# david8862/tf-keras-speech-commands

Hardware: AMD Instinct MI355X
Metric: 1 s@16 kHz clips/sec train-step, simple_cnn bs4096, 1/2/4/8 MI355X; eval top-1 (higher is better)
Workload: dtype f32; 1 GPU; configs[1]: simple_cnn train step = featurize(f32 1 s @16 kHz) + fwd + bwd + Adam, 36 logits (background + 35 words), batch 4096 per GPU; global_batch=4096, parallelism=dp1, gradient_exchange=none (one rank), rccl_ranks=0, library_build=546ca62dfe01

## Files before the change

### tf-keras-speech-commands_amd/csrc/kws_cnn_plan.h

```cpp
#pragma once
#include "kws_model_types.h"
#include "kws_layers.h"
#include "kws_layer1.h"
#include "kws_infer_fused.h"
#include "kws_conv_group.h"
#include "kws_dense_head.h"
#include "kws_conv.h"
#include "kws_conv2_wgrad_fast.h"

namespace kws {

struct CnnPlan {
    bool training, bf16, det;
    bool prepared;
    bool fused_tail;
    bool group;
    bool dense_fused;
    bool l1m;
    bool l1_default_map;
    bool prep_in_stats;
    bool l1_conv2;
    bool compact_g2;
    bool routed_g2;
    bool fuse_pool2;
    bool acc_fwd;
    bool acc_bn2, acc_bn3, acc_bn4;
    bool a3_on_load;
    bool pool4_fused;
    bool wgrad2_bf16;
    bool wgrad2_early;
    bool wgrad2_fast;
    bool l1_fin_in_kernel;
    bool head_bwd_fuses;
    bool fuse_head_fwd;
};

inline CnnPlan plan_cnn(const kws_model *m, int B, int mprec, bool training, bool capturing, bool wants_head_outputs, bool prepared)
{
    const CnnDims &d = m->d;
    CnnPlan p{};
    p.training = training;
    p.bf16 = mprec == 1;
    p.det = m->deterministic != 0;
    p.prepared = !training && prepared;
    const bool split_train = p.bf16 && training;
    const bool default_tail = m->kind == KWS_SIMPLE_CNN && d.H2 == kFuH2 && d.W2 == kFuW2 && d.H3 == kFuH3 && d.W3 == kFuW3;
    p.fused_tail = !training && wants_head_outputs && p.bf16 && default_tail && d.H4 == kFuH4 && d.W4 == kFuW4 && m->C <= kFuHeadCols;
    p.group = split_train && default_tail && (long)blocks_for(B, kFuClips) <= kStatStride;
    p.head_bwd_fuses = head_bwd_fuses(m);
    p.fuse_head_fwd = p.head_bwd_fuses && !p.det;
    p.dense_fused = split_train && m->kind == KWS_SIMPLE_CNN && p.fuse_head_fwd && m->head_K == kDhK && d.flat % (16 * kDhWaves) == 0 && d.flat <= 1024;
    p.l1m = d.H0 % 2 == 0 && d.W0 % 2 == 0 && (d.H0 + 2) * (d.W0 + 2) <= 64 * kL1Stage && (d.H0 / 2) * (d.W0 / 2) <= 4 * kL1MaxTiles;
    p.l1_default_map = d.H0 == 30 && d.W0 == 20;
    p.prep_in_stats = split_train && p.l1m;
    const int P1 = d.H1 * d.W1;
    p.compact_g2 = p.bf16 && P1 * 8 <= 1280 && (size_t)(d.H1 / 2) * (d.W1 / 2) * 32 <= sizeof(float) * (size_t)d.H3 * d.W3 * 64;
    p.routed_g2 = p.compact_g2;
    p.fuse_pool2 = p.group && p.routed_g2 && d.H1 == kGrH1 && d.W1 == kGrW1;
    const bool acc_ok = !p.det && !capturing;
    p.acc_fwd = p.fuse_pool2 && acc_ok;
    p.l1_conv2 = p.prep_in_stats && p.acc_fwd && p.l1_default_map;
    p.a3_on_load = split_train;
    p.pool4_fused = p.acc_fwd && p.dense_fused;
    p.wgrad2_bf16 = p.bf16 && P1 <= 160;
    p.wgrad2_early = p.compact_g2 && p.wgrad2_bf16 && P1 * 8 <= 1280 && P1 * 4 <= 768;
    p.acc_bn2 = p.group && acc_ok && p.routed_g2 && p.wgrad2_early;
    p.acc_bn3 = p.group && acc_ok;
    p.acc_bn4 = p.dense_fused && acc_ok && d.flat == d.H4 * d.W4 * kDhK;
    p.l1_fin_in_kernel = acc_ok && p.l1_default_map;
    p.wgrad2_fast = p.wgrad2_early && p.acc_bn2 && d.H1 == kW2fH && d.W1 == kW2fW;
    return p;
}

}
```

### tf-keras-speech-commands_amd/csrc/kws_conv.h

```cpp
#pragma once
#include "kws_device.h"

namespace kws {

struct ConvGeom {
    int B, H, W, Ho, Wo;
    int stride, pt, pl;
    int KH, KW;
    int pmajor = 0;
};

enum { EPI_NONE = 0, EPI_RELU = 1, EPI_BIAS_RELU6 = 2, EPI_BIAS = 3, EPI_BIAS_RELU = 4,
       EPI_BN_RELU6 = 5,
       EPI_BNBWD_GATE6 = 6 };
enum { MODE_FWD = 0, MODE_DGRAD = 1 };

__host__ __device__ constexpr int stride16(int c) { return (c % 32 == 16) ? c : c + 16; }

template <int CR, int CO, int MODE, int EPI>
__global__ __launch_bounds__(256) void conv_gemm_kernel(const float *__restrict__ src, const float *__restrict__ wgt,
                                                         const float *__restrict__ bias, float *__restrict__ dst,
                                                         ConvGeom g)
{
    constexpr int KC = CR >= 32 ? 32 : CR;
// ... 332 lines not shown
            __syncthreads();
            store_chunk(s1, chunk + 1);
            __syncthreads();
            if (chunk + 3 < nchunks) load_chunk(chunk + 3, s1);
            mma_chunk();
        }
    }

    long mrow[RT][4];
#pragma unroll
    for (int rt = 0; rt < RT; ++rt)
#pragma unroll
        for (int r = 0; r < 4; ++r) {
            const long q = m0 + 16 * (wm * RT + rt) + 4 * lq + r;
            long m = q < M ? q : -1;
            if (pm && q < M) {
                int b, pix;
                row_of(q, b, pix);
                m = (long)b * P + pix;
            }
            mrow[rt][r] = m;
        }
    float ssum[CT], ssq[CT];
#pragma unroll
    for (int c = 0; c < CT; ++c) {
        const int n = 16 * (wn * CT + c) + li;
        float bv = 0.f, sv = 0.f;
        ssum[c] = 0.f; ssq[c] = 0.f;
        if (EPI == EPI_BIAS_RELU6 || EPI == EPI_BIAS || EPI == EPI_BIAS_RELU || EPI == EPI_BN_RELU6) bv = bias[n];
        if (EPI == EPI_BN_RELU6) sv = shift[n];
        float gsc = 0.f, gsh = 0.f, gmean = 0.f, ginv = 0.f;
        if (EPI == EPI_BNBWD_GATE6) { gsc = bias[n]; gsh = bias[CO + n]; gmean = bias[2 * CO + n]; ginv = bias[3 * CO + n]; }
#pragma unroll
        for (int rt = 0; rt < RT; ++rt)
#pragma unroll
            for (int r = 0; r < 4; ++r) {
                const long m = mrow[rt][r];
                if (m >= 0) {
                    float v = acc[rt][c][r];
                    if (EPI == EPI_RELU) v = fmaxf(v, 0.f);
                    if (EPI == EPI_BIAS_RELU6) v = relu6f(v + bv);
                    if (EPI == EPI_BIAS) v = v + bv;
                    if (EPI == EPI_BIAS_RELU) v = fmaxf(v + bv, 0.f);
                    if (EPI == EPI_BN_RELU6) v = relu6f(fmaf(v, bv, sv));
                    if (EPI == EPI_BNBWD_GATE6) {
                        const float zv = shift[m * CO + n], y = fmaf(zv, gsc, gsh);
                        v = (y > 0.f && y < 6.f) ? v : 0.f;
                        dst[m * CO + n] = v;
                        if (STATS) { ssum[c] += v; ssq[c] = fmaf(v, (zv - gmean) * ginv, ssq[c]); }
                        continue;
                    }
                    dst[m * CO + n] = v;
                    if (STATS) { ssum[c] += v; ssq[c] = fmaf(v, v, ssq[c]); }
                }
            }
    }
    if (STATS) {
        __syncthreads();
        double *red = reinterpret_cast<double *>(&As[0][0]);
#pragma unroll
        for (int c = 0; c < CT; ++c) {
            double a = (double)ssum[c], q = (double)ssq[c];
            a += __shfl_xor(a, 16, 64); a += __shfl_xor(a, 32, 64);
            q += __shfl_xor(q, 16, 64); q += __shfl_xor(q, 32, 64);
            const int n = 16 * (wn * CT + c) + li;
            if (lq == 0) { red[(wm * 2 + 0) * CO + n] = a; red[(wm * 2 + 1) * CO + n] = q; }
        }
        __syncthreads();
        for (int i = tid; i < 2 * CO; i += 256) {
            const int which = i / CO, n = i % CO;
            partial[((long)which * CO + n) * partial_stride + blockIdx.x] = red[(0 * 2 + which) * CO + n] + red[(1 * 2 + which) * CO + n];
        }
    }
}

__host__ __device__ constexpr int tr_row_words(int C) { return ((C / 2 / 8) & 1) ? C / 2 : C / 2 + 8; }

typedef short s16x4 __attribute__((ext_vector_type(4)));
__device__ __forceinline__ s16x4 lds_read_tr16(const unsigned char *p)
{
    return __builtin_amdgcn_ds_read_tr16_b64_v4i16((__attribute__((address_space(3))) s16x4 *)(p));
}

template <int CIN, int COUT, int TPB, bool DPRE = false, bool XBN = false>
__global__ __launch_bounds__(256, 2) void conv_wgrad_bf16_kernel(const float *__restrict__ x, const float *__restrict__ dzp,
                                                                  float *__restrict__ dw, const float *__restrict__ zero_page,
                                                                  ConvGeom g, int chunks_per_block, int nranges,
                                                                  Bf16Planes dpl = Bf16Planes{{nullptr, nullptr, nullptr}},
                                                                  const float *__restrict__ xbn = nullptr)
{
    constexpr int KC = 32;
    constexpr int XS = 4 * tr_row_words(CIN), DS = 4 * tr_row_words(COUT);
    constexpr int MT = CIN / 16, NT = COUT / 16, NW = NT / 4;
    constexpr int XU = KC * CIN / 4, DU = KC * COUT / 4;
    constexpr int NXU = XU / 256, NDU = DPRE ? DU / 2 / 256 : DU / 256;
    constexpr int XT = 3 * KC * XS;
    typedef unsigned u32x4 __attribute__((ext_vector_type(4)));
    static_assert(COUT % 64 == 0 && CIN % 32 == 0, "four waves split COUT in 16-column tiles; every thread stages whole units");
    extern __shared__ __attribute__((aligned(16))) unsigned char wsm[];
    unsigned char *Xs = wsm;
    unsigned char *Ds = wsm + TPB * XT;
    const int tid = threadIdx.x, lane = tid & 63, wave = tid >> 6, li = lane & 15, lq = lane >> 4;
    const int HW = g.Ho * g.Wo;
    const long M = (long)g.B * HW;
    const int ngroups = g.KH * g.KW / TPB;
    const int bid = blockIdx.x, tap0 = ((bid >> 3) % ngroups) * TPB, range = (bid / (8 * ngroups)) * 8 + (bid & 7);
    const long nchunk_all = (M + KC - 1) / KC, chunk0 = (long)range * chunks_per_block;
    const int nchunks = (range >= nranges || chunk0 >= nchunk_all) ? 0
                        : (int)(chunk0 + chunks_per_block <= nchunk_all ? chunks_per_block : nchunk_all - chunk0);

    f32x4 acc[TPB][MT][NW];
#pragma unroll
    for (int t = 0; t < TPB; ++t)
#pragma unroll
        for (int mt = 0; mt < MT; ++mt)
#pragma unroll
            for (int nw = 0; nw < NW; ++nw) acc[t][mt][nw] = (f32x4){0.f, 0.f, 0.f, 0.f};

    const float rWo = 1.0f / (float)g.Wo;
    int xb[NXU], xpix[NXU];
#pragma unroll
    for (int j = 0; j < NXU; ++j) {
        const long m = chunk0 * KC + (tid + 256 * j) / (CIN / 4);
        xb[j] = (int)(m / HW); xpix[j] = (int)(m - (long)xb[j] * HW);
    }
    f32x4 sx[TPB][NXU], sd[DPRE ? 1 : NDU];
    u32x4 sdp[DPRE ? 3 : 1][NDU];
    unsigned xok = 0u;
    f32x4 xsc = {0.f, 0.f, 0.f, 0.f}, xsh = {0.f, 0.f, 0.f, 0.f};
    if constexpr (XBN) {
        static_assert(256 % (CIN / 4) == 0 && NXU * TPB <= 32, "one channel group per thread");
        xsc = *reinterpret_cast<const f32x4 *>(xbn + 4 * (tid % (CIN / 4)));
        xsh = *reinterpret_cast<const f32x4 *>(xbn + CIN + 4 * (tid % (CIN / 4)));
    }
    auto load_chunk = [&](int ch) {
        const long m0 = (chunk0 + ch) * KC;
        xok = 0u;
#pragma unroll
        for (int j = 0; j < NXU; ++j) {
            const int e = (tid + 256 * j) % (CIN / 4);
            const int oy = (int)(((float)xpix[j] + 0.5f) * rWo), ox = xpix[j] - oy * g.Wo;
#pragma unroll
            for (int t = 0; t < TPB; ++t) {
                const int tap = tap0 + t, kh = tap / g.KW, kw = tap - kh * g.KW;
                const int sy = oy * g.stride + kh - g.pt, sxx = ox * g.stride + kw - g.pl;
                const bool ok = xb[j] < g.B && sy >= 0 && sy < g.H && sxx >= 0 && sxx < g.W;
                const float *p = ok ? x + (((long)xb[j] * g.H + sy) * g.W + sxx) * CIN + 4 * e : zero_page;
                sx[t][j] = *reinterpret_cast<const f32x4 *>(p);
                if (XBN && ok) xok |= 1u << (j * TPB + t);
            }
            xpix[j] += KC;
            while (xpix[j] >= HW) { xpix[j] -= HW; ++xb[j]; }
        }
#pragma unroll
        for (int j = 0; j < NDU; ++j) {
            const int u = tid + 256 * j;
            if (DPRE) {
                const long m = m0 + u / (COUT / 8);
#pragma unroll
                for (int p = 0; p < 3; ++p)
                    sdp[p][j] = m < M ? *reinterpret_cast<const u32x4 *>(dpl.p[p] + m * COUT + 8 * (u % (COUT / 8))) : (u32x4){0u, 0u, 0u, 0u};
            } else {
                const long m = m0 + u / (COUT / 4);
                const float *p = m < M ? dzp + m * COUT + 4 * (u % (COUT / 4)) : zero_page;
                sd[j] = *reinterpret_cast<const f32x4 *>(p);
            }
        }
    };
    auto store_planes = [&](unsigned char *base, int plane_bytes, int o, f32x4 v) {
        bf16x4 h, m, l;
        split_bf16(v, h, m, l);
        *reinterpret_cast<bf16x4 *>(base + o) = h;
        *reinterpret_cast<bf16x4 *>(base + plane_bytes + o) = m;
        *reinterpret_cast<bf16x4 *>(base + 2 * plane_bytes + o) = l;
    };
    auto store_chunk = [&]() {
#pragma unroll
        for (int j = 0; j < NXU; ++j) {
            const int u = tid + 256 * j, o = (u / (CIN / 4)) * XS + 8 * (u % (CIN / 4));
#pragma unroll
            for (int t = 0; t < TPB; ++t) {
                f32x4 xv = sx[t][j];
                if constexpr (XBN) {
                    if (xok & (1u << (j * TPB + t))) {
#pragma unroll
                        for (int e2 = 0; e2 < 4; ++e2) xv[e2] = relu6f(fmaf(xv[e2], xsc[e2], xsh[e2]));
                    }
                }
                store_planes(Xs + t * XT, KC * XS, o, xv);
            }
        }
#pragma unroll
        for (int j = 0; j < NDU; ++j) {
            const int u = tid + 256 * j;
            if (DPRE) {
                const int o = (u / (COUT / 8)) * DS + 16 * (u % (COUT / 8));
#pragma unroll
                for (int p = 0; p < 3; ++p) *reinterpret_cast<u32x4 *>(Ds + p * KC * DS + o) = sdp[p][j];
            } else {
                store_planes(Ds, KC * DS, (u / (COUT / 4)) * DS + 8 * (u % (COUT / 4)), sd[j]);
            }
        }
    };
    const int trq = li >> 2, trp = li & 3;
    const unsigned char *xfrag = Xs + (4 * lq + trq) * XS + 8 * trp;
    const unsigned char *dfrag = Ds + (4 * lq + trq) * DS + 8 * trp + 32 * (wave * NW);
    auto frag = [&](const unsigned char *base, int stride, int plane, int tile) -> bf16x8 {
        union { struct { s16x4 lo, hi; } s; bf16x8 v; } u;
        u.s.lo = lds_read_tr16(base + plane * KC * stride + 32 * tile);
        u.s.hi = lds_read_tr16(base + plane * KC * stride + 32 * tile + 16 * stride);
        return u.v;
    };

    if (nchunks > 0) load_chunk(0);
    for (int ch = 0; ch < nchunks; ++ch) {
        __syncthreads();
        store_chunk();
        __syncthreads();
        if (ch + 1 < nchunks) load_chunk(ch + 1);
        bf16x8 b[NW][3];
#pragma unroll
        for (int nw = 0; nw < NW; ++nw)
#pragma unroll
            for (int p = 0; p < 3; ++p) b[nw][p] = frag(dfrag, DS, p, nw);
#pragma unroll
        for (int t = 0; t < TPB; ++t)
#pragma unroll
            for (int mt = 0; mt < MT; ++mt) {
                bf16x8 a[3];
#pragma unroll
                for (int p = 0; p < 3; ++p) a[p] = frag(xfrag + t * XT, XS, p, mt);
#pragma unroll
                for (int nw = 0; nw < NW; ++nw) acc[t][mt][nw] = mfma_bf16x6(a, b[nw], acc[t][mt][nw]);
            }
    }
    float *red = reinterpret_cast<float *>(wsm);
#pragma unroll
    for (int t = 0; t < TPB; ++t) {
        __syncthreads();
#pragma unroll
        for (int mt = 0; mt < MT; ++mt)
#pragma unroll
            for (int nw = 0; nw < NW; ++nw)
#pragma unroll
                for (int r = 0; r < 4; ++r) red[(16 * mt + 4 * lq + r) * COUT + 16 * (wave * NW + nw) + li] = acc[t][mt][nw][r];
        __syncthreads();
        if (nchunks > 0)
            for (int i = tid; i < CIN * COUT; i += 256) atomicAdd(dw + (long)(tap0 + t) * CIN * COUT + i, red[i]);
    }
}

template <int N>
__device__ __forceinline__ void load_vec(const float *__restrict__ p, float (&v)[N])
{
    if constexpr (N == 1) {
        v[0] = p[0];
    } else if constexpr (N == 2) {
        const float2 t = *reinterpret_cast<const float2 *>(p);
        v[0] = t.x; v[1] = t.y;
    } else {
#pragma unroll
        for (int i = 0; i < N / 4; ++i) {
            const float4 t = *reinterpret_cast<const float4 *>(p + 4 * i);
            v[4 * i] = t.x; v[4 * i + 1] = t.y; v[4 * i + 2] = t.z; v[4 * i + 3] = t.w;
        }
    }
}

template <int CIN, int COUT, int GPB>
__global__ __launch_bounds__(256) void conv_wgrad_direct_kernel(const float *__restrict__ x, const float *__restrict__ dz,
                                                                 float *__restrict__ dw, const float *__restrict__ zeros,
                                                                 ConvGeom g, int steps_per_wave, LossSumJob job)
{
    constexpr int CB = CIN >= 64 ? 64 : CIN;
    constexpr int CBLK = CIN / CB;
    constexpr int MT = CB / 16, NT = COUT / 16;
    static_assert(CIN % CB == 0 && CB % 16 == 0 && COUT % 16 == 0, "channel counts must be multiples of 16");
    extern __shared__ __attribute__((aligned(16))) float red[];

    if (job.out && blockIdx.x == gridDim.x - 1) {
        if (blockIdx.y == 0) loss_sum_block(job.loss_i, job.correct_i, job.B, job.out, reinterpret_cast<double *>(red));
        return;
    }

    const int lane = threadIdx.x & 63, wave = threadIdx.x >> 6, li = lane & 15, lq = lane >> 4;
    const long M = (long)g.B * g.Ho * g.Wo;
    const int HoWo = g.Ho * g.Wo;
    const int ngroups = g.KH * g.KW * CBLK, grp0 = blockIdx.y * GPB;
    const long step0 = ((long)blockIdx.x * 4 + wave) * steps_per_wave;

    int kh[GPB], kw[GPB], cb[GPB], toff[GPB];
    bool gok[GPB];
#pragma unroll
    for (int gi = 0; gi < GPB; ++gi) {
        const int grp = grp0 + gi, tap = grp / CBLK;
        gok[gi] = grp < ngroups;
        kh[gi] = tap / g.KW;
        kw[gi] = tap % g.KW;
        cb[gi] = (grp % CBLK) * CB;
        toff[gi] = (kh[gi] * g.W + kw[gi]) * CIN + cb[gi];
    }

    f32x4 acc[GPB][MT][NT];
#pragma unroll
    for (int gi = 0; gi < GPB; ++gi)
#pragma unroll
        for (int mt = 0; mt < MT; ++mt)
#pragma unroll
            for (int nt = 0; nt < NT; ++nt) acc[gi][mt][nt] = (f32x4){0.f, 0.f, 0.f, 0.f};

    long p = step0 * 4 + lq;
    int b = (int)(p / HoWo), rem = (int)(p % HoWo), oh = rem / g.Wo, ow = rem % g.Wo;
    auto load_frags = [&](float (&af)[GPB][MT], float (&bf)[NT]) {
        const bool pok = p < M;
        load_vec<NT>(pok ? dz + ((int)p * COUT + NT * li) : zeros + NT * li, bf);
        const int y0 = oh * g.stride - g.pt, x0 = ow * g.stride - g.pl;
        const int base = ((b * g.H + y0) * g.W + x0) * CIN + MT * li;
#pragma unroll
        for (int gi = 0; gi < GPB; ++gi) {
            const bool ok = pok && gok[gi] && (unsigned)(y0 + kh[gi]) < (unsigned)g.H && (unsigned)(x0 + kw[gi]) < (unsigned)g.W;
            load_vec<MT>(ok ? x + (base + toff[gi]) : zeros + MT * li, af[gi]);
        }
        p += 4;
        ow += 4;
        while (ow >= g.Wo) { ow -= g.Wo; ++oh; }
        while (oh >= g.Ho) { oh -= g.Ho; ++b; }
    };
    const long left = (M + 3) / 4 - step0;
    const int nst = left <= 0 ? 0 : (left < steps_per_wave ? (int)left : steps_per_wave);
    float afn[GPB][MT], bfn[NT];
    if (nst > 0) load_frags(afn, bfn);
    for (int st = 0; st < nst; ++st) {
// ... 966 lines not shown
```

### tf-keras-speech-commands_amd/csrc/kws_model.hip

```cpp
#include <cstdlib>
#include <cstring>
#include <string>
#include <type_traits>
#include <vector>

#include "kws_common.h"
#include "kws_model_types.h"
#include "kws_conv.h"
#include "kws_layers.h"
#include "kws_layer1.h"
#include "kws_layer1_moments.h"
#include "kws_layer1_fast.h"
#include "kws_l1_conv2.h"
#include "kws_conv2_wgrad_fast.h"
#include "kws_lite.h"
#include "kws_lite_f16.h"
#include "kws_infer_fused.h"
#include "kws_conv_group.h"
#include "kws_dense_head.h"
#include "kws_cnn_plan.h"

using namespace kws;

namespace {
// ... 104 lines not shown
        w.zmax4 = take(lite ? 0 : as[3] * B);
        w.arg4 = reinterpret_cast<unsigned char *>(take(lite ? 0 : (as[3] * B + 3) / 4));
    }
    w.bytes = off;
    return w;
}

BnCoef coef_of(float *base, int C) { return BnCoef{base, base + C, base + 2 * C, base + 3 * C, base + 4 * C, base + 5 * C}; }
static double *acc_set(ModelRes *R, int pass, int layer, unsigned parity) { return R->acc + ((size_t)(pass * 4 + layer) * 2 + (parity & 1u)) * kAccDoubles; }
static int acc_make_clean(ModelRes *R, hipStream_t s)
{
    if (R->acc_dirty) {
        KWS_HIP_CHECK(hipMemsetAsync(R->acc, 0, sizeof(double) * 2 * 4 * 2 * kAccDoubles, s));
        R->acc_dirty = false;
    }
    return KWS_OK;
}

static int infer_coefs(const kws_model *m, const float *params, const float *state, CnnWs &w, hipStream_t s)
{
    BnInferAll a;
    for (int l = 0; l < 4; ++l) {
        a.C[l] = kCh[l + 1];
        a.gamma[l] = params + m->o_g[l]; a.beta[l] = params + m->o_b[l];
        a.mm[l] = state + m->o_mm[l]; a.mv[l] = state + m->o_mv[l];
        a.k[l] = coef_of(w.coef[l], kCh[l + 1]);
    }
    KWS_LAUNCH("bn_infer_coef_all_kernel", bn_infer_coef_all_kernel, dim3(4), dim3(128), 0, s, a);
    return KWS_OK;
}

inline void stat_grid(long M, int C, int &nblk, int &rows)
{
    const int R = 256 / C;
    long want = (M + (long)R * 8 - 1) / ((long)R * 8);
    nblk = (int)std::min<long>(kMaxStatBlocks, std::max<long>(1, want));
    rows = (int)((M + nblk - 1) / nblk);
    nblk = (int)((M + rows - 1) / rows);
}

template <int CR, int CO, int MODE, int EPI>
int launch_gemm(const float *src, const float *w, const float *bias, float *dst, const ConvGeom &g, hipStream_t s)
{
    const long M = (long)g.B * g.Ho * g.Wo;
    static const std::string name = std::string("conv_gemm_fwd<") + std::to_string(CR) + "," +
                                    std::to_string(CO) + ">";
    KWS_LAUNCH(name.c_str(), (conv_gemm_kernel<CR, CO, MODE, EPI>), dim3(blocks_for(M, 64)), dim3(256), 0, s, src, w, bias, dst, g);
    return KWS_OK;
}

static int cu_count() { return device_cus(); }
template <typename K>
static int resident_blocks(K kernel, int threads, size_t smem)
{
    int nb = 0;
    if (hipOccupancyMaxActiveBlocksPerMultiprocessor(&nb, kernel, threads, smem) != hipSuccess || nb < 1) { (void)hipGetLastError(); nb = 1; }
    return nb;
}

template <int CIN, int COUT, int GPB>
int launch_wgrad(const float *x, const float *dz, float *dw, const ConvGeom &g, hipStream_t s, bool deterministic = false,
                 const LossSumJob *job = nullptr)
{
    const float *zp = zero_page();
    if (!zp) return fail(KWS_ERR_NOMEM, "cannot allocate the zero page on this device");
    constexpr int CB = CIN >= 64 ? 64 : CIN;
    constexpr size_t smem = (4 * 64 * 4 + 16 * COUT) * sizeof(float);
    const long M = (long)g.B * g.Ho * g.Wo;
    const int ngroups = g.KH * g.KW * (CIN / CB), gy = (ngroups + GPB - 1) / GPB;
    const long steps = (M + 3) / 4;
    static const int occ = resident_blocks(conv_wgrad_direct_kernel<CIN, COUT, GPB>, 256, smem);
    const long slots = deterministic ? 1 : std::max<long>(1, (long)cu_count() * occ / gy);
    const long gx_want = std::max<long>(1, std::min<long>(slots, (steps + 4 * 8 - 1) / (4 * 8)));
    const int spw = (int)((steps + 4 * gx_want - 1) / (4 * gx_want));
    const long gx = (steps + 4L * spw - 1) / (4L * spw);
    static const std::string name = "conv_wgrad<" + std::to_string(CIN) + "," + std::to_string(COUT) + ">";
    KWS_LAUNCH(name.c_str(), (conv_wgrad_direct_kernel<CIN, COUT, GPB>), dim3((unsigned)gx + (job ? 1u : 0u), (unsigned)gy), dim3(256), smem,
               s, x, dz, dw, zp, g, spw, job ? *job : LossSumJob{});
    return KWS_OK;
}

template <int CIN, int COUT, int TPB, bool DPRE = false, bool XBN = false>
int launch_wgrad_bf16(const float *x, const float *dz, float *dw, const ConvGeom &g, hipStream_t s, __bf16 *const *dz_planes = nullptr,
                      bool deterministic = false, const float *xbn = nullptr)
{
    if (TPB != 1 && g.KW != TPB) return fail(KWS_ERR_UNSUPPORTED, "split-precision weight gradient expects a kernel %d taps wide", TPB);
    const float *zp = zero_page();
    if (!zp) return fail(KWS_ERR_NOMEM, "cannot allocate the zero page on this device");
    constexpr size_t stage = (size_t)3 * 32 * 4 * (TPB * tr_row_words(CIN) + tr_row_words(COUT)), tile = (size_t)CIN * COUT * sizeof(float);
    constexpr size_t smem = stage > tile ? stage : tile;
    if (int rc = ensure_dynamic_lds(reinterpret_cast<const void *>(conv_wgrad_bf16_kernel<CIN, COUT, TPB, DPRE, XBN>), (int)smem)) return rc;
    static const int occ = resident_blocks(conv_wgrad_bf16_kernel<CIN, COUT, TPB, DPRE, XBN>, 256, smem);
    const long M = (long)g.B * g.Ho * g.Wo, nchunk = (M + 31) / 32;
    const int ngroups = g.KH * g.KW / TPB;
    long nranges = std::max<long>(8, ((long)cu_count() * occ / ngroups) / 8 * 8);
    nranges = std::min<long>(nranges, std::max<long>(8, (nchunk / 4 + 7) / 8 * 8));
    int cpb = (int)((nchunk + nranges - 1) / nranges);
    if (deterministic) { nranges = 8; cpb = (int)nchunk; }
    static const std::string name = "conv_wgrad_bf16<" + std::to_string(CIN) + "," + std::to_string(COUT) + ">";
    const Bf16Planes dpl{{DPRE ? dz_planes[0] : nullptr, DPRE ? dz_planes[1] : nullptr, DPRE ? dz_planes[2] : nullptr}};
    KWS_LAUNCH(name.c_str(), (conv_wgrad_bf16_kernel<CIN, COUT, TPB, DPRE, XBN>), dim3((unsigned)(nranges * ngroups)), dim3(256), smem, s, x, dz, dw,
               zp, g, cpb, (int)nranges, dpl, xbn);
    return KWS_OK;
}

template <int CR, int CO, int MW, int STRIDE>
int launch_dgrad_mw(const float *dz, const float *w, float *dx, const ConvGeom &g, const DgradClasses &cls, int ncls, long max_rows,
                     hipStream_t s)
{
    static const std::string name = "conv_dgrad<" + std::to_string(CR) + "," + std::to_string(CO) + ">";
    const float *zp = zero_page();
    if (!zp) return fail(KWS_ERR_NOMEM, "cannot allocate the zero page on this device");
    KWS_LAUNCH(name.c_str(), (conv_dgrad_direct_kernel<CR, CO, MW, STRIDE>), dim3(blocks_for(max_rows, 64 * MW), (unsigned)ncls), dim3(256), 0, s,
               dz, w, dx, zp, g, cls);
    return KWS_OK;
}

template <int CR, int CO, int STRIDE>
int launch_dgrad(const float *dz, const float *w, float *dx, const ConvGeom &g, hipStream_t s)
{
    if (g.KH > 8 * g.stride || g.KW > 8 * g.stride)
        return fail(KWS_ERR_UNSUPPORTED, "kernel %dx%d too large for the dgrad tap masks (at most %d taps per axis)", g.KH, g.KW, 8 * g.stride);
    DgradClasses cls;
    int ncls = 0;
    long rows[4] = {0, 0, 0, 0}, max_rows = 0;
    for (int cy = 0; cy < g.stride && cy < 2; ++cy)
        for (int cx = 0; cx < g.stride && cx < 2; ++cx) {
            DgradClass c{cy, cx, (g.H - cy + g.stride - 1) / g.stride, (g.W - cx + g.stride - 1) / g.stride};
            if (c.ny <= 0 || c.nx <= 0) continue;
            rows[ncls] = (long)g.B * c.ny * c.nx;
            max_rows = std::max(max_rows, rows[ncls]);
            cls.c[ncls++] = c;
        }
    for (int i = ncls; i < 4; ++i) cls.c[i] = DgradClass{0, 0, 0, 0};
    if (g.stride > 2) return fail(KWS_ERR_UNSUPPORTED, "dgrad is built for strides 1 and 2");
    const long simds = 4L * cu_count();
    int best = 4;
    long best_cost = -1;
    for (int mw = 4; mw >= 1; --mw) {
        long waves = 0;
        for (int i = 0; i < ncls; ++i) waves += ((rows[i] + 15) / 16 + mw - 1) / mw;
        const long cost = ((waves + simds - 1) / simds) * mw;
        if (best_cost < 0 || cost < best_cost) { best_cost = cost; best = mw; }
    }
    switch (best) {
    case 1: return launch_dgrad_mw<CR, CO, 1, STRIDE>(dz, w, dx, g, cls, ncls, max_rows, s);
    case 2: return launch_dgrad_mw<CR, CO, 2, STRIDE>(dz, w, dx, g, cls, ncls, max_rows, s);
    case 3: return launch_dgrad_mw<CR, CO, 3, STRIDE>(dz, w, dx, g, cls, ncls, max_rows, s);
    default: return launch_dgrad_mw<CR, CO, 4, STRIDE>(dz, w, dx, g, cls, ncls, max_rows, s);
    }
}

static int g_matrix_precision = 1;
static inline int matrix_prec(const kws_model *m) { return m->matrix_precision >= 0 ? m->matrix_precision : g_matrix_precision; }
static int g_infer_precision = 0;
static inline int infer_prec(const kws_model *m) { return m->infer_precision >= 0 ? m->infer_precision : g_infer_precision; }

template <int CR, int CO, int MODE, int EPI>
int launch_bf16(const char *what, const float *src, __bf16 *const planes[6], const float *bias, float *dst, const ConvGeom &g_in,
                hipStream_t s, double *partial = nullptr, const float *shift = nullptr, __bf16 *const *src_planes = nullptr,
                const float *abn = nullptr)
{
    ConvGeom g = g_in;
    const long M = MODE == MODE_FWD ? (long)g.B * g.Ho * g.Wo : (long)g.B * g.H * g.W;
    if (M >= (1L << 31)) return fail(KWS_ERR_UNSUPPORTED, "%s: %ld rows exceed the kernel's 32-bit row index", what, M);
    {
        const int P = MODE == MODE_FWD ? g.Ho * g.Wo : g.H * g.W;
        g.pmajor = (g.KH == 3 && g.KW == 3 && P > 1 && P <= 16) ? 1 : 0;
    }
    static const std::string name = std::string(what) + "<" + std::to_string(CR) + "," + std::to_string(CO) + ">";
    const int o = MODE == MODE_FWD ? 3 : 0;
    const Bf16Planes wp{{planes[o], planes[o + 1], planes[o + 2]}};
    constexpr int RT = (MODE == MODE_FWD && CO == 128 && CR == 64) ? 3 : 2;
    const unsigned nblk = blocks_for(M, 32 * RT);
    if (abn) {
        if constexpr (MODE == MODE_FWD && CR == 64 && CO == 128 && EPI == EPI_RELU) {
            if (!partial || (int)nblk > kStatStride || src_planes) return fail(KWS_ERR_UNSUPPORTED, "%s: activation-on-load form needs the fused statistics", what);
            KWS_LAUNCH(name.c_str(), (conv_bf16_kernel<CR, CO, MODE, EPI, RT, true, false, true>), dim3(nblk), dim3(256), 0, s, src, wp, bias, dst, g, partial,
                       kStatStride, nullptr, (Bf16Planes{{nullptr, nullptr, nullptr}}), abn);
            return (int)nblk;
        } else
            return fail(KWS_ERR_UNSUPPORTED, "%s: no activation-on-load form for this layer", what);
    }
// ... 497 lines not shown
    if (P.dense_fused) {
        DenseHeadArgs da{};
        da.a4 = w.a[3]; da.db = params + m->o_db; da.w2 = params + m->o_hk;
        for (int p = 0; p < 3; ++p) { da.fd[p] = w.wsp[2][3 + p]; da.fo[p] = w.wsp[2][p]; }
        da.d1 = w.d1; da.dd1 = w.dd1; da.da4 = w.da4; da.dw2 = grads + m->o_hk; da.db2 = grads + m->o_hb; da.ddb = grads + m->o_db;
        da.B = B; da.C = m->C; da.flat = d.flat;
        if (P.acc_bn4) {
            da.zmax4 = w.zmax4; da.coef4 = coef(3).scale; da.acc4 = acc_set(R, 1, 3, bpar[3]);
            da.drop_rate = drop_rate(); da.seed_lo = slo(); da.seed_hi = shi();
        }
        if (P.pool4_fused) {
            da.z4 = w.z[3]; da.a4w = w.a[3]; da.zmax4w = w.zmax4; da.arg4w = w.arg4; da.H3 = d.H3; da.W3 = d.W3;
            da.in4 = acc_in(3, R->acc_uses[0][3] - 1);
            da.drop_rate = drop_rate(); da.seed_lo = slo(); da.seed_hi = shi();
        }
        da.fw = HeadFwdArgs{params + m->o_hb, a->labels, a->class_weights, a->probs, w.loss_i, w.correct_i, a->grad_scale / (float)B, a->ignore_index};
        const size_t smem = sizeof(float) * (size_t)(16 * (d.flat + 8) + 2 * 16 * kDhKS + 16 * kDhCS + kDhK * kDhCS);
        if (int rc = ensure_dynamic_lds(reinterpret_cast<const void *>(dense_head_fused_kernel), (int)smem)) return rc;
        KWS_LAUNCH("dense_head_fused_kernel", dense_head_fused_kernel, dim3(blocks_for(B, 16)), dim3(kDhThreads), smem, s, da);
    } else if (P.fuse_head_fwd) {
        const HeadFwdArgs hf{params + m->o_hb, a->labels, a->class_weights, a->probs, w.loss_i, w.correct_i, a->grad_scale / (float)B, a->ignore_index};
        KWS_TRY(run_head_bwd(m, B, params, w.d1, nullptr, w.dd1, grads, true, s, grads + m->o_db, nullptr, nullptr, nullptr, false, &hf));
    } else
        KWS_TRY(run_head_bwd(m, B, params, w.d1, w.dlogits, w.dd1, grads, true, s, nullptr, w.loss_i, w.correct_i,
                             stats, P.det));
    const bool fork0_bound = stop_event_bound(fork0_ev);
    if (P.fuse_head_fwd) {
        if (a->forward_event) KWS_HIP_CHECK(hipEventRecord(static_cast<hipEvent_t>(a->forward_event), s));
        if (hook) KWS_TRY(hook->fire(1, s));
    }
    const bool hook_ev_here = hook && hook->wants(2) && hook->ev;
    if (hook) KWS_TRY(hook->fire(2, s, fork0_bound && hook_ev_here));
    if (hook_ev_here) {
        KWS_HIP_CHECK(hipStreamWaitEvent(s2, fork0_ev, 0));
    } else {
        if (!fork0_bound) KWS_HIP_CHECK(hipEventRecord(R->ev[0], s));
        KWS_HIP_CHECK(hipStreamWaitEvent(s2, R->ev[0], 0));
    }
    const LossSumJob sums{w.loss_i, w.correct_i, stats, B};
    KWS_TRY(dense_wgrad(s2, P.det, P.fuse_head_fwd && stats ? &sums : nullptr));
    if (!P.fuse_head_fwd) KWS_TRY(dense_bias_grad());
    if (P.dense_fused) ;
    else if (P.bf16) KWS_TRY_NB(launch_bf16<128, 128, MODE_DGRAD, EPI_NONE>("conv_bf16_dgrad", w.dd1, w.wsp[2], nullptr, w.da4, dense_geom(d, B), s));
    else KWS_TRY(dense_dgrad());
    if (hook) KWS_TRY(hook->fire(3, s));
    return KWS_OK;
}

int CnnCtx::bwd_layer4()
{
    const int C = 128, H = d.H3, W = d.W3;
    const long M = pixels(3);
    const BnCoef k = coef(3);
    const float *gamma = params + m->o_g[3];
    const float rate = drop_rate();
    int nblk, rows;
    stat_grid((long)B * (H / 2) * (W / 2), C, nblk, rows);
    if (P.acc_bn4) ;
    else if (P.bf16)
        KWS_LAUNCH(prof_name("bn_bwd_reduce_pool_kernel", 4), bn_bwd_reduce_routed_full_kernel, dim3(nblk), dim3(256), 0, s, w.zmax4, w.arg4, w.da4, k,
                   w.gz[3], B, H, W, C, rows, w.partial, rate, slo(), shi());
    else KWS_TRY(bwd_reduce_pool(3, H, W, C, w.da4, rate, nblk, rows));
    if (!P.acc_bn4) KWS_TRY(bn_bwd_finalize(3, nblk));
    bwd_arm(3);
    const Bf16PlanesOut dzp{{w.dzp[0], w.dzp[1], w.dzp[2]}};
    if (P.acc_bn4) {
        const unsigned nb = std::min<unsigned>(1024u, blocks_for(M * C / 4, 256));
        if (bn_bwd_walk_ok(M * C / 4, C, nb, kBnRoutedUnits))
            KWS_LAUNCH(prof_name("bn_bwd_apply_planes_kernel", 4), (bn_bwd_apply_routed_planes_kernel<true, true>), dim3(nb), dim3(256), 0, s, w.z[3], w.da4,
                       w.arg4, k, gamma, B, H, W, C, acc_out(3), dzp);
        else
            KWS_LAUNCH(prof_name("bn_bwd_apply_planes_kernel", 4), (bn_bwd_apply_routed_planes_kernel<true, false>), dim3(nb), dim3(256), 0, s, w.z[3], w.da4,
                       w.arg4, k, gamma, B, H, W, C, acc_out(3), dzp);
    } else if (P.bf16)
        KWS_LAUNCH(prof_name("bn_bwd_apply_planes_kernel", 4), bn_bwd_apply_planes_kernel<true>, dim3(blocks_for(M * C / 4, 256)), dim3(256), 0, s,
                   w.z[3], w.gz[3], k, gamma, M * C / 4, C, dzp);
    else KWS_TRY(bn_bwd_apply<true>(3));
    if (hook) KWS_TRY(hook->fire(4, s));
    KWS_TRY(bwd_fork(3));
    const float *in = w.a[2], *kern = params + m->o_k[3];
    float *dk = grads + m->o_k[3];
    const ConvGeom g = geom3x3(B, H, W, 1);
    if (P.bf16 && P.a3_on_load)
        KWS_TRY((launch_wgrad_bf16<64, 128, 1, true, true>(w.z[2], nullptr, dk, g, s2, w.dzp, P.det, coef(2).scale)));
    else if (P.bf16) KWS_TRY(launch_wgrad_bf16<64, 128, 1, true>(in, nullptr, dk, g, s2, w.dzp, P.det));
    else KWS_TRY(launch_wgrad<64, 128, 1>(in, w.gz[3], dk, g, s2, P.det));
    if (a->comm) KWS_TRY(comm_allreduce_early(a->comm, grads + m->o_k[3], m->P - m->o_k[3], s2));
    if (a->bucket_event) KWS_HIP_CHECK(hipEventRecord(static_cast<hipEvent_t>(a->bucket_event), s2));
    if (P.group) {
        fused_bn3_blocks = launch_group_dgrad4(m, B, w, s, P.acc_bn3 ? acc_set(R, 1, 2, bpar[2]) : nullptr);
        if (fused_bn3_blocks < 0) return fused_bn3_blocks;
    } else if (P.bf16 && blocks_for(M, 64) <= (unsigned)kStatStride) {
        const BnCoef k3 = coef(2);
        fused_bn3_blocks = launch_bf16<128, 64, MODE_DGRAD, EPI_BNBWD_GATE6>("conv_bf16_dgrad", nullptr, w.wsp[1], k3.scale, w.gz[2], g, s, w.partial,
                                                                             w.z[2], w.dzp);
        if (fused_bn3_blocks < 0) return fused_bn3_blocks;
    } else if (P.bf16)
        KWS_TRY_NB(launch_bf16<128, 64, MODE_DGRAD, EPI_NONE>("conv_bf16_dgrad", nullptr, w.wsp[1], nullptr, w.da[2], g, s, nullptr, nullptr, w.dzp));
    else KWS_TRY(launch_dgrad<128, 64, 1>(w.gz[3], kern, w.da[2], g, s));
    return KWS_OK;
}

int CnnCtx::bwd_layer3()
{
    const int C = 64, H = d.H3, W = d.W3;
    if (hook) KWS_TRY(hook->fire(5, s));
    const long M = pixels(2);
    const BnCoef k = coef(2);
    const float *gamma = params + m->o_g[2];
    int nblk, rows;
    stat_grid(M, C, nblk, rows);
    if (fused_bn3_blocks > 0) nblk = fused_bn3_blocks;
    else
        KWS_LAUNCH(prof_name("bn_bwd_reduce_kernel", 3), bn_bwd_reduce_kernel<false>, dim3(nblk), dim3(256), 0, s, w.z[2], w.da[2], k, w.gz[2], B, H, W, C,
                   rows, w.partial, 0.f, slo(), shi());
    if (!P.acc_bn3) KWS_TRY(bn_bwd_finalize(2, nblk));
    bwd_arm(2);
    if (P.acc_bn3)
        KWS_LAUNCH(prof_name("bn_bwd_apply_kernel", 3), bn_bwd_apply_acc_kernel<false>, dim3(std::min<unsigned>(1024u, blocks_for(M * C / 4, 256))), dim3(256), 0, s,
                   w.z[2], w.gz[2], k, gamma, M * C / 4, C, acc_out(2));
    else KWS_TRY(bn_bwd_apply<false>(2));
    KWS_TRY(bwd_fork(2));
    const float *in = w.a[1], *kern = params + m->o_k[2];
    float *dk = grads + m->o_k[2];
    const ConvGeom g = geom3x3(B, d.H2, d.W2, 2);
    if (P.bf16) KWS_TRY(launch_wgrad_bf16<32, 64, 3>(in, w.gz[2], dk, g, s2, nullptr, P.det));
    else KWS_TRY(launch_wgrad<32, 64, 3>(in, w.gz[2], dk, g, s2, P.det));
    if (P.group) {
        if (P.acc_bn2) bwd_arm(1);
        KWS_TRY(launch_group_dgrad3(m, B, w, s, P.acc_bn2 ? acc_set(R, 1, 1, bpar[1]) : nullptr));
    }
    else KWS_TRY(launch_dgrad<64, 32, 2>(w.gz[2], kern, w.da[1], g, s));
    return KWS_OK;
}

int CnnCtx::bwd_layer2()
{
    const int C = 32, H1 = d.H1, W1 = d.W1;
    const long M = pixels(1);
    const BnCoef k = coef(1);
    const long NW = (long)B * (H1 / 2) * (W1 / 2);
    int nblk, rows;
    stat_grid(NW, C, nblk, rows);
    if (P.acc_bn2) ;
    else if (P.compact_g2 && P.routed_g2)
        KWS_LAUNCH(prof_name("bn_bwd_reduce_pool_kernel", 2), bn_bwd_reduce_routed_kernel, dim3(nblk), dim3(256), 0, s, w.zmax2, w.da[1], k, NW, C,
                   rows, w.partial);
    else if (P.compact_g2)
        KWS_LAUNCH(prof_name("bn_bwd_reduce_pool_kernel", 2), bn_bwd_reduce_pool_kernel<true>, dim3(nblk), dim3(256), 0, s, w.z[1], w.da[1], k,
                   w.gz[1], B, H1, W1, C, rows, w.partial, 0.f, slo(), shi(), reinterpret_cast<unsigned char *>(w.da[2]));
    else KWS_TRY(bwd_reduce_pool(1, H1, W1, C, w.da[1], 0.f, nblk, rows));
    if (!P.acc_bn2) {
        if (P.wgrad2_early) bwd_arm(1);
        KWS_TRY(bn_bwd_finalize(1, nblk));
    }
    const float *in = w.a[0], *kern = params + m->o_k[1];
    float *dk = grads + m->o_k[1];
    const Conv2Clip cc = conv2_clip(d, B);
    BnBwdArgs bn = {w.z[1], params + m->o_g[1], k.mean, k.inv, k.k2, k.k3};
    if (P.compact_g2) { bn.gw = w.da[1]; bn.arg = P.routed_g2 ? w.arg2 : reinterpret_cast<const unsigned char *>(w.da[2]); }
    BnBwdArgs bn_w = bn;
    if (P.acc_bn2) {
        bn.acc = bn_w.acc = acc_set(R, 1, 1, bpar[1]);
        bn.M = bn_w.M = M;
        bn.acc_clear_set = acc_set(R, 1, 1, bpar[1] + 1);
        bn.dgamma = grads + m->o_g[1]; bn.dbeta = grads + m->o_b[1]; bn.k2w = k.k2; bn.k3w = k.k3;
    }
    auto wgrad_grid = [&](int occ) { return dim3(P.det ? 1u : cc.even_grid(cu_count() * std::min(occ, 2))); };
// ... 735 lines not shown
```

Measured before the change: 8.026 million clips/s.

## Add position-major conv4 weight-gradient schedule that skips out-of-bounds taps

Adds a position-major variant of the split-bf16 weight-gradient kernel for small output maps (at most 16 positions). Each block is assigned one tap and walks only the output positions whose input for that tap lies inside the image. Block slots are shared out across taps in proportion to their number of valid positions, so padded positions are never loaded or multiplied. The cost is extra indexing logic, a host-side planning routine, and atomic accumulation across more blocks per tap.

Measured after the change: 8.222 million clips/s (median of 6 runs). 1.02x the previous value.

```diff
diff --git a/tf-keras-speech-commands_amd/csrc/kws_cnn_plan.h b/tf-keras-speech-commands_amd/csrc/kws_cnn_plan.h
--- a/tf-keras-speech-commands_amd/csrc/kws_cnn_plan.h
+++ b/tf-keras-speech-commands_amd/csrc/kws_cnn_plan.h
@@ -27,6 +27,7 @@
     bool acc_bn2, acc_bn3, acc_bn4;
     bool a3_on_load;
     bool pool4_fused;
+    bool wgrad_pmajor;
     bool wgrad2_bf16;
     bool wgrad2_early;
     bool wgrad2_fast;
@@ -62,6 +63,7 @@
     p.l1_conv2 = p.prep_in_stats && p.acc_fwd && p.l1_default_map;
     p.a3_on_load = split_train;
     p.pool4_fused = p.acc_fwd && p.dense_fused;
+    p.wgrad_pmajor = split_train && !p.det && d.H3 * d.W3 <= 16;
     p.wgrad2_bf16 = p.bf16 && P1 <= 160;
     p.wgrad2_early = p.compact_g2 && p.wgrad2_bf16 && P1 * 8 <= 1280 && P1 * 4 <= 768;
     p.acc_bn2 = p.group && acc_ok && p.routed_g2 && p.wgrad2_early;
diff --git a/tf-keras-speech-commands_amd/csrc/kws_conv.h b/tf-keras-speech-commands_amd/csrc/kws_conv.h
--- a/tf-keras-speech-commands_amd/csrc/kws_conv.h
+++ b/tf-keras-speech-commands_amd/csrc/kws_conv.h
@@ -438,14 +438,21 @@
     return __builtin_amdgcn_ds_read_tr16_b64_v4i16((__attribute__((address_space(3))) s16x4 *)(p));
 }
 
-template <int CIN, int COUT, int TPB, bool DPRE = false, bool XBN = false>
+struct WgradPm {
+    unsigned long long pos[9];
+    int npos[9];
+    int slot0[10];
+};
+
+template <int CIN, int COUT, int TPB, bool DPRE = false, bool XBN = false, bool PM = false>
 __global__ __launch_bounds__(256, 2) void conv_wgrad_bf16_kernel(const float *__restrict__ x, const float *__restrict__ dzp,
                                                                   float *__restrict__ dw, const float *__restrict__ zero_page,
                                                                   ConvGeom g, int chunks_per_block, int nranges,
                                                                   Bf16Planes dpl = Bf16Planes{{nullptr, nullptr, nullptr}},
-                                                                  const float *__restrict__ xbn = nullptr)
+                                                                  const float *__restrict__ xbn = nullptr, WgradPm pm = WgradPm{})
 {
     constexpr int KC = 32;
+    static_assert(!PM || TPB == 1, "the position-major form is built and measured for one tap per block");
     constexpr int XS = 4 * tr_row_words(CIN), DS = 4 * tr_row_words(COUT);
     constexpr int MT = CIN / 16, NT = COUT / 16, NW = NT / 4;
     constexpr int XU = KC * CIN / 4, DU = KC * COUT / 4;
@@ -460,10 +467,34 @@
     const int HW = g.Ho * g.Wo;
     const long M = (long)g.B * HW;
     const int ngroups = g.KH * g.KW / TPB;
-    const int bid = blockIdx.x, tap0 = ((bid >> 3) % ngroups) * TPB, range = (bid / (8 * ngroups)) * 8 + (bid & 7);
-    const long nchunk_all = (M + KC - 1) / KC, chunk0 = (long)range * chunks_per_block;
-    const int nchunks = (range >= nranges || chunk0 >= nchunk_all) ? 0
-                        : (int)(chunk0 + chunks_per_block <= nchunk_all ? chunks_per_block : nchunk_all - chunk0);
+    const int bid = blockIdx.x;
+    int tap0, nchunks;
+    long chunk0 = 0;
+    int pm_cc = 0, pm_pi = 0, pm_np = 1, pm_dcc = 0, pm_dpi = 0;
+    unsigned long long pm_pos = 0ull;
+    unsigned ld_taps = 0u, st_taps = 0u;
+    if constexpr (PM) {
+        const int xcd = bid & 7, slot = bid >> 3;
+        int grp = 0;
+        while (grp + 1 < ngroups && slot >= pm.slot0[grp + 1]) ++grp;
+        tap0 = grp * TPB;
+        pm_np = pm.npos[grp]; pm_pos = pm.pos[grp];
+        const int nclip = (g.B + KC - 1) / KC, c0 = (int)((long)xcd * nclip / 8), c1 = (int)((long)(xcd + 1) * nclip / 8);
+        const int k = slot - pm.slot0[grp], ns = pm.slot0[grp + 1] - pm.slot0[grp];
+        const int items = (c1 - c0) * pm_np;
+        nchunks = (k < ns && pm_np > 0 && items > k) ? (items - k + ns - 1) / ns : 0;
+        if (nchunks > 0) {
+            pm_cc = c0 + k / pm_np; pm_pi = k % pm_np;
+            pm_dcc = ns / pm_np; pm_dpi = ns % pm_np;
+        }
+    } else {
+        tap0 = ((bid >> 3) % ngroups) * TPB;
+        const int range = (bid / (8 * ngroups)) * 8 + (bid & 7);
+        const long nchunk_all = (M + KC - 1) / KC;
+        chunk0 = (long)range * chunks_per_block;
+        nchunks = (range >= nranges || chunk0 >= nchunk_all) ? 0
+                  : (int)(chunk0 + chunks_per_block <= nchunk_all ? chunks_per_block : nchunk_all - chunk0);
+    }
 
     f32x4 acc[TPB][MT][NW];
 #pragma unroll
@@ -489,7 +520,47 @@
         xsc = *reinterpret_cast<const f32x4 *>(xbn + 4 * (tid % (CIN / 4)));
         xsh = *reinterpret_cast<const f32x4 *>(xbn + CIN + 4 * (tid % (CIN / 4)));
     }
+    auto load_chunk_pm = [&]() {
+        const int pos = (int)(pm_pos >> (4 * pm_pi)) & 15, oy = pos / g.Wo, ox = pos - oy * g.Wo;
+        const int b0 = pm_cc * KC;
+        ld_taps = (1u << TPB) - 1u;
+        xok = 0u;
+#pragma unroll
+        for (int t = 0; t < TPB; ++t) {
+            const int tap = tap0 + t, kh = tap / g.KW, kw = tap - kh * g.KW;
+            const int sy = oy * g.stride + kh - g.pt, sxx = ox * g.stride + kw - g.pl;
+            if (sy >= 0 && sy < g.H && sxx >= 0 && sxx < g.W) {
+#pragma unroll
+                for (int j = 0; j < NXU; ++j) {
+                    const int u = tid + 256 * j, b = b0 + u / (CIN / 4);
+                    const float *p = b < g.B ? x + (((long)b * g.H + sy) * g.W + sxx) * CIN + 4 * (u % (CIN / 4)) : zero_page;
+                    sx[t][j] = *reinterpret_cast<const f32x4 *>(p);
+                    if (XBN && b < g.B) xok |= 1u << (j * TPB + t);
+                }
+            } else {
+                ld_taps &= ~(1u << t);
+            }
+        }
+#pragma unroll
+        for (int j = 0; j < NDU; ++j) {
+            const int u = tid + 256 * j;
+            if (DPRE) {
+                const int b = b0 + u / (COUT / 8);
+                const long m = (long)b * HW + pos;
+#pragma unroll
+                for (int p = 0; p < 3; ++p)
+                    sdp[p][j] = b < g.B ? *reinterpret_cast<const u32x4 *>(dpl.p[p] + m * COUT + 8 * (u % (COUT / 8))) : (u32x4){0u, 0u, 0u, 0u};
+            } else {
+                const int b = b0 + u / (COUT / 4);
+                const float *p = b < g.B ? dzp + ((long)b * HW + pos) * COUT + 4 * (u % (COUT / 4)) : zero_page;
+                sd[j] = *reinterpret_cast<const f32x4 *>(p);
+            }
+        }
+        pm_cc += pm_dcc; pm_pi += pm_dpi;
+        if (pm_pi >= pm_np) { pm_pi -= pm_np; ++pm_cc; }
+    };
     auto load_chunk = [&](int ch) {
+        if constexpr (PM) { load_chunk_pm(); return; }
         const long m0 = (chunk0 + ch) * KC;
         xok = 0u;
 #pragma unroll
@@ -536,6 +607,7 @@
             const int u = tid + 256 * j, o = (u / (CIN / 4)) * XS + 8 * (u % (CIN / 4));
 #pragma unroll
             for (int t = 0; t < TPB; ++t) {
+                if (PM && !((st_taps >> t) & 1u)) continue;
                 f32x4 xv = sx[t][j];
                 if constexpr (XBN) {
                     if (xok & (1u << (j * TPB + t))) {
@@ -571,6 +643,7 @@
     if (nchunks > 0) load_chunk(0);
     for (int ch = 0; ch < nchunks; ++ch) {
         __syncthreads();
+        st_taps = ld_taps;
         store_chunk();
         __syncthreads();
         if (ch + 1 < nchunks) load_chunk(ch + 1);
@@ -580,7 +653,8 @@
 #pragma unroll
             for (int p = 0; p < 3; ++p) b[nw][p] = frag(dfrag, DS, p, nw);
 #pragma unroll
-        for (int t = 0; t < TPB; ++t)
+        for (int t = 0; t < TPB; ++t) {
+            if (PM && !((st_taps >> t) & 1u)) continue;
 #pragma unroll
             for (int mt = 0; mt < MT; ++mt) {
                 bf16x8 a[3];
@@ -589,6 +663,7 @@
 #pragma unroll
                 for (int nw = 0; nw < NW; ++nw) acc[t][mt][nw] = mfma_bf16x6(a, b[nw], acc[t][mt][nw]);
             }
+        }
     }
     float *red = reinterpret_cast<float *>(wsm);
 #pragma unroll
@@ -604,6 +679,50 @@
         if (nchunks > 0)
             for (int i = tid; i < CIN * COUT; i += 256) atomicAdd(dw + (long)(tap0 + t) * CIN * COUT + i, red[i]);
     }
+}
+
+inline bool wgrad_pm_plan(const ConvGeom &g, int max_slots, int min_chunks, WgradPm &pm)
+{
+    const int P = g.Ho * g.Wo, ntaps = g.KH * g.KW;
+    if (P < 1 || P > 16 || ntaps < 1 || ntaps > 9) return false;
+    long w[9], wsum = 0;
+    int live = 0;
+    for (int tap = 0; tap < ntaps; ++tap) {
+        const int kh = tap / g.KW, kw = tap % g.KW;
+        pm.pos[tap] = 0ull; pm.npos[tap] = 0;
+        for (int p = 0; p < P; ++p) {
+            const int sy = (p / g.Wo) * g.stride + kh - g.pt, sx = (p % g.Wo) * g.stride + kw - g.pl;
+            if (sy < 0 || sy >= g.H || sx < 0 || sx >= g.W) continue;
+            pm.pos[tap] |= (unsigned long long)p << (4 * pm.npos[tap]);
+            ++pm.npos[tap];
+        }
+        w[tap] = pm.npos[tap]; wsum += w[tap]; live += w[tap] > 0;
+    }
+    if (live < 1 || max_slots < live) return false;
+    const long nclip = ((long)g.B + 31) / 32, want = (wsum * nclip + 8L * min_chunks - 1) / (8L * min_chunks);
+    const int S = (int)(want < live ? live : want > max_slots ? max_slots : want);
+    int s[9], total = 0;
+    for (int tap = 0; tap < ntaps; ++tap) {
+        s[tap] = w[tap] ? (int)((long)S * w[tap] / wsum) : 0;
+        if (w[tap] && s[tap] < 1) s[tap] = 1;
+        total += s[tap];
+    }
+    for (; total < S; ++total) {
+        int best = -1;
+        for (int tap = 0; tap < ntaps; ++tap)
+            if (w[tap] && (best < 0 || w[tap] * s[best] > w[best] * s[tap])) best = tap;
+        ++s[best];
+    }
+    for (; total > S; --total) {
+        int best = -1;
+        for (int tap = 0; tap < ntaps; ++tap)
+            if (s[tap] > 1 && (best < 0 || w[tap] * s[best] <= w[best] * s[tap])) best = tap;
+        --s[best];
+    }
+    pm.slot0[0] = 0;
+    for (int tap = 0; tap < ntaps; ++tap) pm.slot0[tap + 1] = pm.slot0[tap] + s[tap];
+    for (int tap = ntaps + 1; tap < 10; ++tap) pm.slot0[tap] = pm.slot0[ntaps];
+    return true;
 }
 
 template <int N>
diff --git a/tf-keras-speech-commands_amd/csrc/kws_model.hip b/tf-keras-speech-commands_amd/csrc/kws_model.hip
--- a/tf-keras-speech-commands_amd/csrc/kws_model.hip
+++ b/tf-keras-speech-commands_amd/csrc/kws_model.hip
@@ -210,7 +210,7 @@
 
 template <int CIN, int COUT, int TPB, bool DPRE = false, bool XBN = false>
 int launch_wgrad_bf16(const float *x, const float *dz, float *dw, const ConvGeom &g, hipStream_t s, __bf16 *const *dz_planes = nullptr,
-                      bool deterministic = false, const float *xbn = nullptr)
+                      bool deterministic = false, const float *xbn = nullptr, bool pmajor = false)
 {
     if (TPB != 1 && g.KW != TPB) return fail(KWS_ERR_UNSUPPORTED, "split-precision weight gradient expects a kernel %d taps wide", TPB);
     const float *zp = zero_page();
@@ -227,6 +227,19 @@
     if (deterministic) { nranges = 8; cpb = (int)nchunk; }
     static const std::string name = "conv_wgrad_bf16<" + std::to_string(CIN) + "," + std::to_string(COUT) + ">";
     const Bf16Planes dpl{{DPRE ? dz_planes[0] : nullptr, DPRE ? dz_planes[1] : nullptr, DPRE ? dz_planes[2] : nullptr}};
+    if (pmajor && TPB != 1) return fail(KWS_ERR_UNSUPPORTED, "the position-major weight gradient takes one tap per block");
+    if constexpr (TPB == 1) {
+        if (pmajor) {
+            if (int rc = ensure_dynamic_lds(reinterpret_cast<const void *>(conv_wgrad_bf16_kernel<CIN, COUT, 1, DPRE, XBN, true>), (int)smem)) return rc;
+            static const int occ_pm = resident_blocks(conv_wgrad_bf16_kernel<CIN, COUT, 1, DPRE, XBN, true>, 256, smem);
+            WgradPm pm{};
+            if (!wgrad_pm_plan(g, cu_count() * occ_pm / 8, 4, pm))
+                return fail(KWS_ERR_UNSUPPORTED, "position-major weight gradient: a %d x %d map on %d block slots", g.Ho, g.Wo, cu_count() * occ_pm);
+            KWS_LAUNCH(name.c_str(), (conv_wgrad_bf16_kernel<CIN, COUT, 1, DPRE, XBN, true>), dim3(8u * (unsigned)pm.slot0[ngroups]), dim3(256), smem, s, x,
+                       dz, dw, zp, g, 0, 0, dpl, xbn, pm);
+            return KWS_OK;
+        }
+    }
     KWS_LAUNCH(name.c_str(), (conv_wgrad_bf16_kernel<CIN, COUT, TPB, DPRE, XBN>), dim3((unsigned)(nranges * ngroups)), dim3(256), smem, s, x, dz, dw,
                zp, g, cpb, (int)nranges, dpl, xbn);
     return KWS_OK;
@@ -890,8 +903,8 @@
     float *dk = grads + m->o_k[3];
     const ConvGeom g = geom3x3(B, H, W, 1);
     if (P.bf16 && P.a3_on_load)
-        KWS_TRY((launch_wgrad_bf16<64, 128, 1, true, true>(w.z[2], nullptr, dk, g, s2, w.dzp, P.det, coef(2).scale)));
-    else if (P.bf16) KWS_TRY(launch_wgrad_bf16<64, 128, 1, true>(in, nullptr, dk, g, s2, w.dzp, P.det));
+        KWS_TRY((launch_wgrad_bf16<64, 128, 1, true, true>(w.z[2], nullptr, dk, g, s2, w.dzp, P.det, coef(2).scale, P.wgrad_pmajor)));
+    else if (P.bf16) KWS_TRY(launch_wgrad_bf16<64, 128, 1, true>(in, nullptr, dk, g, s2, w.dzp, P.det, nullptr, P.wgrad_pmajor));
     else KWS_TRY(launch_wgrad<64, 128, 1>(in, w.gz[3], dk, g, s2, P.det));
     if (a->comm) KWS_TRY(comm_allreduce_early(a->comm, grads + m->o_k[3], m->P - m->o_k[3], s2));
     if (a->bucket_event) KWS_HIP_CHECK(hipEventRecord(static_cast<hipEvent_t>(a->bucket_event), s2));
```
